# kosta777/parallel-genomeseq

Measured on AMD Instinct MI355X. Metric: GCUPS (cell updates/s), 150 bp reads vs 50 Mbp reference, whole job (score + argmax + traceback), higher is better.
Workload: dtype f16

## Files before the change

include/mi355_sw.h:

```cpp
#ifndef MI355_SW_H_
#define MI355_SW_H_

#include <stddef.h>
#include <stdint.h>

#ifdef __cplusplus
extern "C" {
#endif

enum { MI355_SW_F32 = 0, MI355_SW_U8SAT = 1 };

enum {
  MI355_SW_OK = 0,
  MI355_SW_EINVAL = -22,
  MI355_SW_ENOMEM = -12,
  MI355_SW_ENODEV = -19,
  MI355_SW_ENOTSUP = -95,
  MI355_SW_ERANGE = -34
};

enum {
  MI355_SW_SCORE_ONLY = 1
};

// ... 148 lines not shown
int mi355_sw_fill_matrix(mi355_sw_ctx *ctx, const char *x, size_t nx, const char *y, size_t ny,
                         const mi355_sw_params *params, float *H);

int mi355_sw_argmax(mi355_sw_ctx *ctx, const char *x, size_t nx, const char *y, size_t ny,
                    const mi355_sw_params *params, int64_t *index_x, int64_t *index_y, float *max);

int mi355_sw_last_timings(const mi355_sw_ctx *ctx, double out[6]);

int mi355_sw_last_counters(const mi355_sw_ctx *ctx, uint64_t out[4]);
int mi355_sw_last_counter(const mi355_sw_ctx *ctx, const char *name, uint64_t *out);

int mi355_sw_prefix_values(mi355_sw_ctx *ctx, float *values, size_t capacity, size_t *n_sub);

int mi355_sw_prefix_thin_items(mi355_sw_ctx *ctx, size_t n_items, const uint32_t *items, int P, int P2, int64_t sub_len, int64_t left, int64_t right,
                               const mi355_sw_params *params, float *values, size_t capacity, size_t *n_per_item);

int mi355_sw_seed_usable(const uint8_t *read, int32_t len, int k, const uint8_t *letters, size_t n_letters);
int mi355_sw_seed_certify_ok(int64_t d, int64_t smax, int64_t g, int64_t u);
int mi355_sw_seed_certify_window(int64_t start, int64_t m, int64_t d, int64_t smax, int64_t g, int64_t n, int64_t *lo, int64_t *hi);
int mi355_sw_seed_k(int letters, int min_len, int64_t n);
uint32_t mi355_sw_seed_hash(const uint8_t *codes, int k);
int mi355_sw_seed_cluster(size_t n_hits, const int64_t *starts, const int32_t *offsets, int64_t width, int64_t *lo, int64_t *hi, int *distinct);
int mi355_sw_seed_hits(mi355_sw_ctx *ctx, int64_t left, int64_t right, int k, uint32_t *counts, int64_t *starts, int32_t *offsets, int *k_used);

const char *mi355_sw_last_path(const mi355_sw_ctx *ctx);

enum {
  MI355_SW_CELL_I16 = 0,
  MI355_SW_CELL_U8 = 1,
  MI355_SW_CELL_F32 = 2,
  MI355_SW_CELL_F32U8 = 3,
  MI355_SW_CELL_F16 = 4,
  MI355_SW_CELL_U8H = 5
};
typedef struct {
  int cell;
  int lanes;
  int rows_per_lane;
  int strips;
  int twin;
  int64_t chunk_len;
  int64_t sub_len;
  int64_t warm;
  double cells;
  double valu_ops_per_cell;
  char name[160];
// ... 33 lines not shown
```

parallel-genomeseq_amd/capi.py:

```python
import ctypes as C
import os
import time

import numpy as np

_HERE = os.path.dirname(os.path.abspath(__file__))
LIB_PATH = os.path.join(_HERE, "libmi355_sw.so")

F32, U8SAT = 0, 1
SCORE_ONLY = 1

EXPORTS = [
    "mi355_sw_create", "mi355_sw_destroy", "mi355_sw_last_error", "mi355_sw_default_params",
    "mi355_sw_align", "mi355_sw_set_reference", "mi355_sw_align_batch", "mi355_sw_batch_upload",
    "mi355_sw_batch_run", "mi355_sw_score_ranges", "mi355_sw_align_scored_range", "mi355_sw_align_split", "mi355_sw_make_string_range", "mi355_sw_fill_matrix",
    "mi355_sw_argmax", "mi355_sw_true2raw", "mi355_sw_raw2true", "mi355_sw_last_timings", "mi355_sw_free_result", "mi355_sw_free_results",
    "mi355_sw_build_info", "mi355_sw_last_kernel", "mi355_sw_batch_run_view",
    "mi355_sw_multi_create", "mi355_sw_multi_destroy", "mi355_sw_multi_last_error", "mi355_sw_multi_device_count",
    "mi355_sw_multi_rccl_version", "mi355_sw_multi_align_split", "mi355_sw_multi_set_reference",
    "mi355_sw_multi_align_batch", "mi355_sw_multi_last_timings",
    "mi355_sw_set_option", "mi355_sw_option_names", "mi355_sw_multi_set_option", "mi355_sw_last_counters", "mi355_sw_last_counter", "mi355_sw_batch_upload_packed", "mi355_sw_best_range", "mi355_sw_last_path",
    "mi355_sw_default_affine_params", "mi355_sw_affine_align", "mi355_sw_affine_batch_run", "mi355_sw_affine_score_ranges",
    "mi355_sw_affine_align_trace", "mi355_sw_affine_batch_trace", "mi355_sw_affine_pairs_run", "mi355_sw_affine_pairs_trace",
    "mi355_sw_prefix_values", "mi355_sw_prefix_thin_items", "mi355_sw_affine_pairs_run_mode", "mi355_sw_affine_pairs_trace_mode",
    "mi355_sw_affine_pairs_run_band", "mi355_sw_affine_pairs_trace_band",
    "mi355_sw_affine_extend_run", "mi355_sw_affine_extend_trace",
    "mi355_sw_affine_extend_run_band", "mi355_sw_affine_extend_trace_band",
    "mi355_sw_affine_global_run", "mi355_sw_affine_global_trace",
    "mi355_sw_affine_extend_run_zdrop", "mi355_sw_affine_extend_trace_zdrop",
    "mi355_sw_seed_k", "mi355_sw_seed_hash", "mi355_sw_seed_cluster", "mi355_sw_seed_hits",
    "mi355_sw_seed_usable", "mi355_sw_seed_certify_ok", "mi355_sw_seed_certify_window",
]
SEED_HIT_CAP = 32
AFFINE_LOCAL, AFFINE_END_TO_END = 0, 1
AFFINE_MODES = {"local": AFFINE_LOCAL, "end_to_end": AFFINE_END_TO_END}
MULTI_RCCL = 1


class Params(C.Structure):
    _fields_ = [("lut", C.POINTER(C.c_float)), ("match", C.c_float), ("mismatch", C.c_float),
                ("gap", C.c_float), ("semantics", C.c_int)]


class AffineParams(C.Structure):
    _fields_ = [("lut", C.POINTER(C.c_float)), ("match", C.c_float), ("mismatch", C.c_float),
                ("gap_open", C.c_float), ("gap_extend", C.c_float)]


class ExtendList(C.Structure):
    _fields_ = [("npairs", C.c_size_t), ("query", C.POINTER(C.c_int32)), ("q_lo", C.POINTER(C.c_int32)), ("q_hi", C.POINTER(C.c_int32)),
                ("lefts", C.POINTER(C.c_int64)), ("rights", C.POINTER(C.c_int64)), ("backward", C.POINTER(C.c_uint8))]


class Result(C.Structure):
# ... 26 lines not shown

class MI355Error(RuntimeError):
    def __init__(self, code, msg):
        super().__init__("mi355_sw error %d: %s" % (code, msg))
        self.code = code


_LIB = None


def lib():
    global _LIB
    if _LIB is None:
        if not os.path.exists(LIB_PATH):
            raise ImportError("libmi355_sw.so not built: run `python -c 'import __graft_entry__ as g; g.build()'` "
                              "or `make -C parallel-genomeseq_amd/csrc`")
        L = C.CDLL(LIB_PATH)
        L.mi355_sw_last_error.restype = C.c_char_p
        L.mi355_sw_build_info.restype = C.c_char_p
        L.mi355_sw_multi_last_error.restype = C.c_char_p
        L.mi355_sw_option_names.restype = C.c_char_p
        L.mi355_sw_last_path.restype = C.c_char_p
        L.mi355_sw_seed_hash.restype = C.c_uint32
        for name in EXPORTS:
            getattr(L, name)
        _LIB = L
    return _LIB


def make_params(semantics=F32, match=3.0, mismatch=-3.0, gap=2.0, lut=None):
    p = Params()
    keep = None
    if lut is not None:
        keep = np.ascontiguousarray(lut, dtype=np.float32).reshape(65536)
        p.lut = keep.ctypes.data_as(C.POINTER(C.c_float))
    p.match, p.mismatch, p.gap, p.semantics = match, mismatch, gap, semantics
    return p, keep


def make_affine_params(match=3.0, mismatch=-3.0, gap_open=5.0, gap_extend=1.0, lut=None):
    p = AffineParams()
    keep = None
    if lut is not None:
        keep = np.ascontiguousarray(lut, dtype=np.float32).reshape(65536)
        p.lut = keep.ctypes.data_as(C.POINTER(C.c_float))
    p.match, p.mismatch, p.gap_open, p.gap_extend = match, mismatch, gap_open, gap_extend
# ... 477 lines not shown
            out[k] = np.array([r[k] for r in rows], dtype=np.int64)
        for k in ("cons_x", "cons_y", "cigar"):
            out[k] = [r[k] for r in rows]
        return out

    def align_batch(self, xs, y=None, **kw):
        if y is not None:
            self.set_reference(y)
        self.batch_upload(xs)
        return self.batch_run(**kw)

    def last_timings(self):
        t = (C.c_double * 6)()
        self._L.mi355_sw_last_timings(self._ctx, t)
        return dict(score_us=t[0], locate_us=t[1], trace_us=t[2], total_us=t[3], score_launches=int(t[4]), cells=t[5])


    def last_counters(self):
        c = (C.c_uint64 * 4)()
        self._L.mi355_sw_last_counters(self._ctx, c)
        out = dict(requeried=int(c[0]), whole_batch_again=int(c[1]), candidates=int(c[2]), left_window=int(c[3]))
        for name in ("first_settled", "saved_locates", "saved_traces", "saved_fallbacks", "walk_widened", "wait_retries", "early_settled", "beyond_f16", "prefix_certified",
                     "prefix_second_pass", "prefix_thinned", "prefix_thin_items", "pooled_loops", "prefix_seeded", "prefix_seed_hits", "prefix_calibrated", "seed_certified",
                     "zdrop_stopped", "zdrop_rows_run", "exact_launches", "trace_launches"):
            v = C.c_uint64(0)
            rc = self._L.mi355_sw_last_counter(self._ctx, name.encode(), C.byref(v))
            if rc:
                raise MI355Error(rc, "mi355_sw_last_counter(%s)" % name)
            out[name] = int(v.value)
        return out

    def prefix_values(self):
        nsub = C.c_size_t(0)
        self._chk(self._L.mi355_sw_prefix_values(self._ctx, None, C.c_size_t(0), C.byref(nsub)))
        if nsub.value == 0:
            return None
        out = np.zeros((self._nbatch, nsub.value), dtype=np.float32)
        self._chk(self._L.mi355_sw_prefix_values(self._ctx, out.ctypes.data_as(C.POINTER(C.c_float)), C.c_size_t(out.size), C.byref(nsub)))
        return out

    def prefix_thin_items(self, items, P, left, right, P2=38, sub_len=256, semantics=F32, match=3.0, mismatch=-3.0, gap=2.0, lut=None):
        p, keep = make_params(semantics, match, mismatch, gap, lut)
        flat = np.ascontiguousarray(np.asarray(items, dtype=np.uint32).reshape(-1, 2))
        per = C.c_size_t(0)
        args = (self._ctx, C.c_size_t(len(flat)), flat.ctypes.data_as(C.POINTER(C.c_uint32)), C.c_int(P), C.c_int(P2), C.c_int64(sub_len),
                C.c_int64(left), C.c_int64(right), C.byref(p))
        self._chk(self._L.mi355_sw_prefix_thin_items(*args, None, C.c_size_t(0), C.byref(per)))
# ... 141 lines not shown
def seed_usable(read, k, letters=b"ACGT"):
    x = np.ascontiguousarray(np.frombuffer(bytes(read), dtype=np.uint8))
    a = np.ascontiguousarray(np.frombuffer(bytes(letters), dtype=np.uint8))
    rc = lib().mi355_sw_seed_usable(x.ctypes.data_as(C.POINTER(C.c_uint8)), C.c_int32(len(x)), C.c_int(k),
                                    a.ctypes.data_as(C.POINTER(C.c_uint8)), C.c_size_t(len(a)))
    if rc < 0:
        raise MI355Error(rc, "mi355_sw_seed_usable")
    return int(rc)


def seed_certify_ok(d, smax, g, u):
    return bool(lib().mi355_sw_seed_certify_ok(C.c_int64(d), C.c_int64(smax), C.c_int64(g), C.c_int64(u)))


def seed_certify_window(start, m, d, smax, g, n):
    lo, hi = C.c_int64(0), C.c_int64(0)
    rc = lib().mi355_sw_seed_certify_window(C.c_int64(start), C.c_int64(m), C.c_int64(d), C.c_int64(smax), C.c_int64(g), C.c_int64(n),
                                            C.byref(lo), C.byref(hi))
    if rc < 0:
        raise MI355Error(rc, "mi355_sw_seed_certify_window")
    return (lo.value, hi.value) if rc == 1 else None


def seed_cluster(hits, width):
    starts = np.ascontiguousarray([h[0] for h in hits], dtype=np.int64)
    offs = np.ascontiguousarray([h[1] for h in hits], dtype=np.int32)
    lo, hi, d = C.c_int64(0), C.c_int64(0), C.c_int(0)
    rc = lib().mi355_sw_seed_cluster(C.c_size_t(len(starts)), starts.ctypes.data_as(C.POINTER(C.c_int64)), offs.ctypes.data_as(C.POINTER(C.c_int32)),
                                     C.c_int64(width), C.byref(lo), C.byref(hi), C.byref(d))
    if rc < 0:
        raise MI355Error(rc, "mi355_sw_seed_cluster")
    return (lo.value, hi.value, d.value) if rc == 1 else None
```

parallel-genomeseq_amd/csrc/host_common.h:

```cpp
namespace {

constexpr size_t kProfileLdsMax = 120 * 1024;
constexpr int kMaxRowsFast = 512;
constexpr size_t kDirsBudget = 16ull << 30;
constexpr size_t kExactLdsMax = 159 * 1024;

#define MI355_SW_BOOL_OPTIONS(X) \
  X(no_f16) X(no_unsat) X(no_sample) X(no_satflag) X(no_solo) X(no_wave) X(no_comb) X(no_twin) X(no_wide) X(no_strip) \
  X(no_quant) X(no_devlist) X(no_ref_cache) X(no_strip_groups) X(u8_long_twin) X(long_twin) X(no_long) \
  X(no_requery) X(force_f32) X(no_long_p32) X(no_opt_margin) X(no_wave_prof) X(no_wave_window) X(no_first) X(no_long_save) X(u8_sample_short) X(no_wave_pieces) X(no_u8_early) X(no_wave_f16) X(no_devlist_by_id) X(no_f16_mirror) X(no_f16m_int_diag) X(no_affine_sweep) X(no_affine_prof) X(no_affine_pairs) X(no_prefix) X(trace) \
  X(no_prefix_low) X(no_prefix_cascade) X(no_prefix_step) X(no_affine_band) X(no_prefix_thin) X(no_prefix_seed) X(no_seed_certify)
#define MI355_SW_INT_OPTIONS(X) X(strip_r) X(slot) X(few_r) X(chunk) X(long_pipes) X(long_wgs) X(long_sub) X(long_r) X(long_groups) X(assume_cus) X(long_save_what) X(prefix_min_cols) X(prefix_thin_min_cols) X(prefix_seed_min_cols) X(seed_certify_min_cols) X(seed_ride)
struct Options {
#define X(n) bool n = false;
  MI355_SW_BOOL_OPTIONS(X)
#undef X
#define X(n) long n = 0;
  MI355_SW_INT_OPTIONS(X)
#undef X
  bool prefix_tiles = false;
  long prefix_rowp = 0;
  long prefix_rowp_step = 0;
  bool prefix_thin_items = false;
  int fault_inject = 0;
};
inline std::string option_env_name(const char *n) {
  std::string e = "MI355_SW_";
  for (const char *c = n; *c; ++c) e += (char)std::toupper((unsigned char)*c);
  return e;
}
inline Options options_from_env() {
  Options o;
#define X(n) o.n = std::getenv(option_env_name(#n).c_str()) != nullptr;
  MI355_SW_BOOL_OPTIONS(X)
#undef X
// ... 292 lines not shown
  std::vector<uint16_t> h_atab;
  DevBuf aprof;
  std::vector<float> h_aprof;
  DevBuf rev_codes, rev_bytes, rev_q;
  bool rev_ref_valid = false, rev_q_valid = false;
  uint64_t rev_ref_version = 0, rev_q_version = 0;
  size_t rev_q_total = 0;
  std::vector<uint8_t> h_pieces;
  size_t saved_locates = 0, saved_traces = 0, saved_fallbacks = 0;
  size_t walk_widened = 0;
  size_t zdrop_stopped = 0;
  size_t zdrop_rows_run = 0;
  size_t exact_launches = 0;
  size_t trace_launches = 0;
  DevBuf thin_items, thin_out, thin_vals;
  DevBuf seed_tab, seed_hits;
  std::vector<uint8_t> h_qbytes;
  const void *h_qbytes_of = nullptr;
  uint64_t h_qbytes_version = 0;
  QueryBatch calib_q;
  PrefixBackground pbg;
  size_t prefix_seeded = 0;
  size_t seed_certified = 0;
  size_t prefix_seed_hits = 0;
  size_t prefix_calibrated = 0;
  DevBuf pkeys, pthr, psel, psel2, qcnt, sel2, gcnt, wlut, ckpt, first, keys, ranges, stab, ftab, ftab_s, htab, htab8, soloblk, flags, submax, lut, probs, dirs, outs_f, outs_i, cons, walkp, hmat, brow, wprobs, scan;
  std::vector<int64_t> h_ranges;
  std::vector<int16_t> h_stab;
  std::vector<float> h_ftab, h_ftab_s;
  int fshift = 0;
  std::vector<uint16_t> h_htab, h_htab8;
  std::vector<hipEvent_t> score_ev;
  size_t score_ev_used = 0;
  std::vector<std::vector<char>> arenas;
  PinBuf pin_probs, pin_walk, pin_out, pin_solo_up, pin_solo_down;
  std::vector<PinBuf> pin_cons;
  size_t cons_used = 0;
  double timings[6] = {0, 0, 0, 0, 0, 0};
  Options opts;
  ViewStore view;
  ScoredRanges scored;
  Helpers helpers;
  mi355_sw_kernel_info last_kernel = {};
};

namespace {

struct OptScope {
  const Options *prev;
  const DevInfo *prev_dev;
  explicit OptScope(const mi355_sw_ctx *c) : prev(tl_opt), prev_dev(tl_dev) {
    if (!prev) tl_pooled_loops = 0;
    if (c) { tl_opt = &c->opts; tl_dev = &c->dev; }
  }
  ~OptScope() { tl_opt = prev; tl_dev = prev_dev; if (!prev) tl_no_wait = false; }
};
// ... 430 lines not shown
```

parallel-genomeseq_amd/csrc/host_pipeline.h:

```cpp
namespace {

void set_result(mi355_sw_result &r, float score, int64_t ix, int64_t iy, const TraceOut *t) {
  r.score = score;
  r.end_x = score > 0 ? ix : 0;
  r.end_y = score > 0 ? iy : 0;
  r.pos = t ? t->pos : 0;
  const size_t len = t ? t->len : 0;
  r.cons_len = len;
  r.cons_x = (char *)malloc(2 * len + 2);
  r.cons_y = r.cons_x + len + 1;
  if (len) { memcpy(r.cons_x, t->cx, len); memcpy(r.cons_y, t->cy, len); }
  r.cons_x[len] = 0;
  r.cons_y[len] = 0;
}

int trace_located(mi355_sw_ctx *ctx, const RefData &ref, const QueryBatch &q, const Range &rg,
                  const mi355_sw_params &p, const std::vector<int64_t> &qwarm, const ScoreTable &table,
                  const std::vector<int> &qidx, const std::vector<Located> &loc, std::vector<TraceOut> &tout) {
  tout.assign(qidx.size(), TraceOut());
  const Margin mg = table.margin(q.maxlen);
  const float slope = (float)mg.slope();
  auto row_need = [&](int64_t i) { return mg.finite() ? clamp_cols((double)i + std::ceil((double)i * (double)slope) + 2.0) : kColsMax; };
  std::vector<size_t> todo;
  const bool wave_ok = wave_scoring_ok(p) && !opt().no_wave;
// ... 1879 lines not shown
  for (size_t k = 0; k < nq; ++k) if (!qfast[k]) slow.push_back((int)k);
  for (size_t r = 0; r < nr && !slow.empty(); ++r) {
    std::vector<Located> loc;
    std::vector<TraceOut> t;
    int rc = exact_full(ctx, ref, q, ranges[r], p, slow, false, loc, t);
    if (rc) return rc;
    for (size_t i = 0; i < slow.size(); ++i) maxima[r * nq + slow[i]] = loc[i].score;
  }
  sc.valid = keep;
  return 0;
}

int check_params(mi355_sw_ctx *ctx, const mi355_sw_params *p) {
  if (!ctx) return MI355_SW_EINVAL;
  if (!p) return fail(ctx, MI355_SW_EINVAL, "params is NULL");
  if (p->semantics != MI355_SW_F32 && p->semantics != MI355_SW_U8SAT) return fail(ctx, MI355_SW_EINVAL, "unknown semantics");
  return 0;
}

void reset_timings(mi355_sw_ctx *ctx) {
  for (double &t : ctx->timings) t = 0;
  ctx->score_ev_used = 0; ctx->arenas.clear(); ctx->cons_used = 0;
  ctx->last_kernel = mi355_sw_kernel_info{};
  ctx->requeried = 0; ctx->whole_again = 0; ctx->candidates = 0; ctx->prefix_certified = 0; ctx->prefix_second_pass = 0; ctx->prefix_thinned = 0; ctx->prefix_thin_items = 0; ctx->prefix_seeded = 0; ctx->prefix_seed_hits = 0; ctx->seed_certified = 0; ctx->prefix_calibrated = 0; ctx->prefix_named = false; ctx->left_window = 0; ctx->beyond_f16 = 0; ctx->first_settled = 0;
  ctx->hook_ids.clear(); ctx->hook_nsub = 0;
  ctx->saved_locates = 0; ctx->saved_traces = 0; ctx->saved_fallbacks = 0; ctx->walk_widened = 0; ctx->wait_retries = 0; ctx->early_settled = 0;
  ctx->zdrop_stopped = 0; ctx->zdrop_rows_run = 0;
  ctx->exact_launches = 0; ctx->trace_launches = 0;
  ctx->path.clear();
}

void reset_after_decline(mi355_sw_ctx *ctx) {
  const std::string ran = ctx->path;
  reset_timings(ctx);
  ctx->path = ran;
}

}
```

parallel-genomeseq_amd/csrc/host_score.h:

```cpp
namespace {

struct ScoreTable {
  bool ok = false;
  bool integral = false;
  std::string why;
  int gap = 0, smax = 0;
  float gapf = 0, smaxf = 0;
  std::vector<int16_t> stab;
  std::vector<uint16_t> htab;
  std::vector<uint16_t> htab8;
  std::vector<float> ftab;
  Margin margin(double rows) const { return make_margin(smaxf, gapf, integral, rows); }
};

struct Bucket {
  int first = 0, count = 0;
  int maxlen = 0;
  int R = 0;
  int SL = 16;
  int sem = kSemI16;
  bool strips = false;
  bool twin = false;
  bool comb = false;
  bool unsat = false;
// ... 348 lines not shown
  return true;
}

double valu_ops_per_cell(const Bucket &b) {
  const int R = b.R;
  const double over = b.SL == 8 ? 4.0 : 3.0;
  double per_step;
  int cells_per_row = 2;
  const int folded = b.sampled ? (R + sample_rows(b) - 1) / sample_rows(b) : R;
  double fold = (b.sampled ? 1.0 / kScoreMK : 1.0) * ((folded + 1) / 2);
  if (b.prefix && b.rowp && b.step) fold = 1.0;
  switch (b.sem) {
    case kSemF32:   per_step = 3.0 * R + (b.longp ? (b.sampled ? 1.0 / kLongMK : 1.0) * ((R + 1) / 2) : fold) + 1 + over; cells_per_row = 1; break;
    case kSemF32U8: per_step = 6.0 * R + (R + 1) / 2 + over; cells_per_row = 1; break;
    case kSemF16:   per_step = 3.0 * R + fold + 1 + over; break;
    case kSemU8H:   { const int odd = R / 2; per_step = 4.0 * R + odd / 2 + odd % 2 + R % 2 + over; break; }
    case kSemU8:    per_step = 5.0 * R + (R + 1) / 2 + R % 2 + over; break;
    default:        per_step = 4.0 * R + (R + 1) / 2 + R % 2 + over; break;
  }
  if (b.twin && !b.comb) per_step += R;
  return per_step / (double)(cells_per_row * R);
}

int launch_score(const ScoreInst &want, dim3 grid, size_t shmem, hipStream_t st, const ScoreArgs &a) {
  for (size_t k = 0; k < kScoreInsts.size(); ++k) {
    if (!(kScoreInsts[k] == want)) continue;
    if (shmem > 48 * 1024)
      (void)hipFuncSetAttribute(reinterpret_cast<const void *>(kScoreKernels[k]), hipFuncAttributeMaxDynamicSharedMemorySize, (int)shmem);
    hipLaunchKernelGGL(kScoreKernels[k], grid, dim3(256), shmem, st, a);
    return 0;
  }
  for (size_t k = 0; low_step_inst(want) && k < std::size(kR2Step); ++k) {
    if (kR2Step[k] != want.R) continue;
    if (shmem > 48 * 1024)
      (void)hipFuncSetAttribute(reinterpret_cast<const void *>(kLowStepKernels[k]), hipFuncAttributeMaxDynamicSharedMemorySize, (int)shmem);
    hipLaunchKernelGGL(kLowStepKernels[k], grid, dim3(256), shmem, st, a);
    return 0;
  }
  return -1;
}

int kernel_sem(const Bucket &b) {
  if (b.sem == kSemF16 && b.mirror) return opt().no_f16m_int_diag ? kSemF16MF : kSemF16M;
  return b.sem;
}

constexpr int64_t kPrefixMinCols = (int64_t)8 << 20;
constexpr int kPrefixProbe = 64;
inline int64_t prefix_cols_min() { const long v = opt().prefix_min_cols; return v > 0 ? (int64_t)v : kPrefixMinCols; }
float prefix_bound(const ScoreTable &t, int m, int P, float slack, bool rowp) {
  const float b = (float)t.smax * (float)(m - P) + slack;
  return rowp ? std::max(b, (float)t.smax * (float)P) : b;
}
bool prefix_height_ok(const ScoreTable &t, const Bucket &b, int minlen, int R, bool rowp, bool step = false) {
  const int P = kPrefixLanes * R;
  if (!(rowp && step ? prefix_step_listed(R) : listed(kR8M, R)) || minlen <= P) return false;
  return (float)t.smax * (float)minlen > prefix_bound(t, b.maxlen, P, rowp ? rowp_slack(t, rowp_mk(step)) : sample_slack(t, b), rowp);
}
bool prefix_ok(const ScoreTable &t, const Bucket &b, int minlen, int64_t n, const mi355_sw_params &p) {
  if (opt().no_prefix || p.semantics != MI355_SW_F32 || !t.integral || t.gap <= 0 || t.smax <= 0) return false;
  if (!(b.fast && b.sem == kSemF16 && b.mirror && b.sampled && !b.strips && !b.twin && !b.satflag && !b.unsat && b.SL == 8 && b.count >= 2)) return false;
  if (kernel_sem(b) != kSemF16M || !listed(kR8M, b.R)) return false;
// ... 91 lines not shown
    };
    auto cost = [&](int64_t c) { return rounds(c) * (double)(c + warm + SL); };
    const double r0 = rounds(cl);
    if (r0 <= 8.0) {
      const double need_rounds = std::min(2.0, r0);
      const double base = cost(cl);
      int64_t best = cl;
      double best_gain = 0.0;
      const int64_t lo = std::max<int64_t>({quant, floor_cl, (cl / 2 + quant - 1) / quant * quant});
      for (int64_t c = lo; c <= 2 * cl; c += quant) {
        const double rc = rounds(c);
        if (rc < need_rounds) continue;
        const double gain = 1.0 - cost(c) / base;
        if (gain < (rc < r0 ? 0.07 : 0.04)) continue;
        if (gain > best_gain) { best_gain = gain; best = c; }
      }
      cl = best;
    }
  }
  { const long v = opt().chunk; if (v >= 64) cl = v / 64 * 64; }
  return cl;
}

int score_tables(mi355_sw_ctx *ctx, int maxlen, int64_t maxrange, const ScoreTable &t) {
  const void *stab_was = ctx->stab.p, *ftab_was = ctx->ftab.p;
  if (ctx->stab.ensure(t.stab.size() * 2) || ctx->ftab.ensure(t.ftab.size() * 4 + 16))
    return fail(ctx, MI355_SW_ENOMEM, "hipMalloc(score scratch) failed");
  if (ctx->stab.p != stab_was || ctx->h_stab != t.stab) {
    ctx->h_stab = t.stab;
    HIPCHK(ctx, hipMemcpyAsync(ctx->stab.p, ctx->h_stab.data(), ctx->h_stab.size() * 2, hipMemcpyHostToDevice, ctx->stream));
  }
  if (!t.ftab.empty() && (ctx->ftab.p != ftab_was || ctx->h_ftab != t.ftab)) {
    ctx->h_ftab = t.ftab;
    HIPCHK(ctx, hipMemcpyAsync(ctx->ftab.p, ctx->h_ftab.data(), ctx->h_ftab.size() * 4, hipMemcpyHostToDevice, ctx->stream));
  }
  if (!t.ftab.empty()) {
    const double bound = (double)t.smaxf * (double)std::min<int64_t>(std::max(1, maxlen), std::max<int64_t>(1, maxrange)) + (double)t.smaxf + 1.0;
    ctx->fshift = std::max(1, std::min(100, std::ilogb(bound) + 2));
    std::vector<float> scaled(t.ftab.size());
    for (size_t k = 0; k < scaled.size(); ++k) scaled[k] = std::ldexp(t.ftab[k], -ctx->fshift);
    const void *was = ctx->ftab_s.p;
    if (ctx->ftab_s.ensure(scaled.size() * 4 + 16)) return fail(ctx, MI355_SW_ENOMEM, "hipMalloc(score scratch) failed");
    if (ctx->ftab_s.p != was || ctx->h_ftab_s != scaled) {
      ctx->h_ftab_s.swap(scaled);
      HIPCHK(ctx, hipMemcpyAsync(ctx->ftab_s.p, ctx->h_ftab_s.data(), ctx->h_ftab_s.size() * 4, hipMemcpyHostToDevice, ctx->stream));
    }
// ... 223 lines not shown
  }
  return 0;
}

int score_launch(mi355_sw_ctx *ctx, const RefData &ref, const QueryBatch &q, const std::vector<Range> &ranges,
                 const mi355_sw_params &p, const ScoreTable &t, Bucket &b, const ScoreIO *io = nullptr) {
  if (b.longp && io == nullptr) return long_score_launch(ctx, ref, q, ranges, p, t, b);
  HostTrace trace_("score_launch");
  const size_t nr = ranges.size();
  int64_t maxlen = 0;
  for (auto &r : ranges) maxlen = std::max(maxlen, r.hi - r.lo);
  const int sem = kernel_sem(b);
  const CellLaunch cl = cell_launch(ctx, t, sem);
  const int nqw = b.twin ? 1 : cl.queries;
  const size_t npairs = nqw == 1 ? (size_t)b.count : ((size_t)b.count + 1) / 2;
  b.sub_len = score_sub_len(p.semantics, b);
  const bool free_sub = p.semantics == MI355_SW_F32 && b.strips;
  if (b.strips && !free_sub) {
    const int64_t cl0 = pick_chunk_len(maxlen, npairs * nr, b.warm, b.SL, b.twin, b.maxlen, b.sub_len, 0);
    while (2 * cl0 / b.sub_len > 64) b.sub_len *= 2;
  }
  const bool chain_main = b.prefix && b.rowp && b.step && b.SL == kPrefixLanes && (b.bulk || (!b.second && b.count >= kPrefixChain - kPrefixProbe));
  b.chunk_len = pick_chunk_len(maxlen, npairs * nr, b.warm, b.SL, b.twin, b.maxlen, b.sub_len, free_sub ? 64 * kSeg : b.sub_len, chain_main);
  if (free_sub && b.chunk_len % (64 * kSeg) == 0) b.sub_len = b.chunk_len / 64;
  if (b.strips) while (b.chunk_len / b.sub_len > 64) b.sub_len *= 2;
  if (b.sub_len > b.chunk_len || b.chunk_len % b.sub_len != 0) b.sub_len = b.chunk_len;
  const int64_t cpr = (maxlen + b.chunk_len - 1) / b.chunk_len;
  const int nslot = 256 / b.SL;
  const int64_t cgroups = ((b.twin ? (cpr + 1) / 2 : cpr) + nslot - 1) / nslot;
  if ((double)npairs * (double)cgroups > 2.0e9) return fail(ctx, MI355_SW_ENOTSUP, "grid too large");

  ScoreArgs a;
  a.refcodes = ref.codes.as<uint8_t>();
  a.ref_len = (int64_t)ref.n;
  a.range_lo = io ? io->range_lo : ctx->ranges.as<int64_t>();
  a.range_hi = io ? io->range_hi : ctx->ranges.as<int64_t>() + nr;
  a.chunk_len = b.chunk_len;
  a.sub_len = b.sub_len;
  a.warm = (cpr == 1) ? 0 : b.warm;
  if (b.prefix && !b.strips && a.warm > 0) {
    const Margin pmg = t.margin(b.SL * b.R);
    if (pmg.finite()) a.warm = std::min(a.warm, (pmg.cols(b.SL * b.R) + 63) / 64 * 64);
  }
  a.chunks_per_range = (int)cpr;
  a.qbytes = q.bytes.as<uint8_t>();
  a.qoff = q.offs.as<int64_t>();
  a.qlen = q.lens.as<int32_t>();
  a.qsel = q.sel.as<int32_t>();
  a.qfirst = b.first;
  a.qcount = b.count;
  a.nq = (int)q.nq;
  a.stab = cl.tab;
  a.ncodes = ref.ncodes;
  a.gap2 = cl.gap2;
  a.clamp2 = 255u * 0x00010001u;
  a.pubmax = b.unsat ? cl.pubmax : 0u;
  a.keys = io ? io->keys : ctx->keys.as<unsigned long long>();
  a.flag_count = nullptr; a.flag_list = nullptr; a.flag_cap = 0; a.flag_value = 0;
  a.submax_out = nullptr; a.submax_stride = 0;
  if (b.sampled && nr != 1) b.sampled = false;
  if (b.satflag) {
    a.flag_count = ctx->flags.as<unsigned int>();
    a.flag_list = reinterpret_cast<uint2 *>(ctx->flags.as<unsigned int>() + 2);
    a.flag_cap = ctx->flag_cap;
    a.flag_value = (uint32_t)half_bits(1.0f);
  }
// ... 128 lines not shown
    case kKeyF32:       memcpy(&v, &hi, 4); return v;
    default:            return (float)hi;
  }
}

constexpr int kRetryNoWait = 1;

int score_fetch(mi355_sw_ctx *ctx, size_t count, std::vector<unsigned long long> &keys, const void *from = nullptr) {
  keys.resize(count);
  HIPCHK(ctx, hipMemcpyAsync(keys.data(), from ? from : ctx->keys.p, count * 8, hipMemcpyDeviceToHost, ctx->stream));
  int32_t long_status = 0;
  if (ctx->long_launched) HIPCHK(ctx, hipMemcpyAsync(&long_status, ctx->flags.as<unsigned int>() + 1, 4, hipMemcpyDeviceToHost, ctx->stream));
  HIPCHK(ctx, hipStreamSynchronize(ctx->stream));
  ctx->long_launched = false;
  if (long_status != 0) {
    ctx->score_ev_used = 0;
    if (!tl_no_wait) { tl_no_wait = true; ctx->wait_retries += 1; return kRetryNoWait; }
    return fail(ctx, MI355_SW_ENODEV, "sw_long_kernel: a pipeline wait expired (a wavefront of the workgroup made no progress)");
  }
  for (size_t e = 0; e + 1 < ctx->score_ev_used; e += 2) {
    float ms = 0;
    HIPCHK(ctx, hipEventElapsedTime(&ms, ctx->score_ev[e], ctx->score_ev[e + 1]));
    ctx->timings[0] += (double)ms * 1000.0;
  }
  ctx->score_ev_used = 0;
  return 0;
}

}
```

parallel-genomeseq_amd/csrc/mi355_sw.hip:

```cpp
#include "../../include/mi355_sw.h"

#include <hip/hip_runtime.h>

#include <algorithm>
#include <array>
#include <atomic>
#include <chrono>
#include <condition_variable>
#include <functional>
#include <iterator>
#include <map>
#include <future>
#include <mutex>
#include <thread>
#include <memory>
#include <cmath>
#include <cstdarg>
#include <cstdio>
#include <cstdlib>
#include <cstring>
#include <string>
#include <utility>
#include <vector>

// ... 723 lines not shown
  return 0;
}

int mi355_sw_last_counters(const mi355_sw_ctx *ctx, uint64_t out[4]) {
  if (!ctx || !out) return MI355_SW_EINVAL;
  out[0] = ctx->requeried; out[1] = ctx->whole_again; out[2] = ctx->candidates; out[3] = ctx->left_window;
  return 0;
}

int mi355_sw_last_counter(const mi355_sw_ctx *ctx, const char *name, uint64_t *out) {
  if (!ctx || !name || !out) return MI355_SW_EINVAL;
  const std::string k(name);
  if (k == "requeried") *out = ctx->requeried;
  else if (k == "whole_batch_again") *out = ctx->whole_again;
  else if (k == "candidates") *out = ctx->candidates;
  else if (k == "prefix_certified") *out = ctx->prefix_certified;
  else if (k == "prefix_second_pass") *out = ctx->prefix_second_pass;
  else if (k == "prefix_thinned") *out = ctx->prefix_thinned;
  else if (k == "prefix_thin_items") *out = ctx->prefix_thin_items;
  else if (k == "prefix_seeded") *out = ctx->prefix_seeded;
  else if (k == "prefix_seed_hits") *out = ctx->prefix_seed_hits;
  else if (k == "seed_certified") *out = ctx->seed_certified;
  else if (k == "prefix_calibrated") *out = ctx->prefix_calibrated;
  else if (k == "left_window") *out = ctx->left_window;
  else if (k == "beyond_f16") *out = ctx->beyond_f16;
  else if (k == "first_settled") *out = ctx->first_settled;
  else if (k == "wait_retries") *out = ctx->wait_retries;
  else if (k == "early_settled") *out = ctx->early_settled;
  else if (k == "saved_locates") *out = ctx->saved_locates;
  else if (k == "saved_traces") *out = ctx->saved_traces;
  else if (k == "saved_fallbacks") *out = ctx->saved_fallbacks;
  else if (k == "walk_widened") *out = ctx->walk_widened;
  else if (k == "zdrop_stopped") *out = ctx->zdrop_stopped;
  else if (k == "zdrop_rows_run") *out = ctx->zdrop_rows_run;
  else if (k == "exact_launches") *out = ctx->exact_launches;
  else if (k == "trace_launches") *out = ctx->trace_launches;
  else if (k == "pooled_loops") *out = tl_pooled_loops;
  else return MI355_SW_EINVAL;
  return 0;
}

int mi355_sw_prefix_values(mi355_sw_ctx *ctx, float *values, size_t capacity, size_t *n_sub) {
  if (!ctx || !n_sub) return MI355_SW_EINVAL;
  OptScope opt_scope_(ctx);
  const size_t nsub = (size_t)ctx->hook_nsub, nq = ctx->batch.nq;
  *n_sub = nsub;
// ... 55 lines not shown
  if ((n_hits && (!starts || !offsets)) || !lo || !hi || !distinct || width < 0) return MI355_SW_EINVAL;
  std::vector<SeedHit> hits(n_hits);
  for (size_t k = 0; k < n_hits; ++k) hits[k] = SeedHit{starts[k], offsets[k]};
  *lo = 0; *hi = 0; *distinct = 0;
  return seed_cluster(hits, width, *lo, *hi, *distinct) ? 1 : 0;
}

int mi355_sw_seed_usable(const uint8_t *read, int32_t len, int k, const uint8_t *letters, size_t n_letters) {
  if (!read || len < 0 || k < 1 || k > kSeedMaxK || (n_letters && !letters)) return MI355_SW_EINVAL;
  int code_of[256];
  for (int b = 0; b < 256; ++b) code_of[b] = -1;
  for (size_t i = 0; i < n_letters; ++i) code_of[letters[i]] = 0;
  const int64_t off = 0;
  const int32_t id = 0;
  SeedTable t;
  if (!seed_table_build(t, k, read, &off, &len, &id, 1, code_of)) return MI355_SW_ENOTSUP;
  std::vector<uint32_t> u;
  seed_usable(t, 1, u);
  return (int)u[0];
}

int mi355_sw_seed_certify_ok(int64_t d, int64_t smax, int64_t g, int64_t u) { return seed_certify_ok(d, smax, g, u) ? 1 : 0; }

int mi355_sw_seed_certify_window(int64_t start, int64_t m, int64_t d, int64_t smax, int64_t g, int64_t n, int64_t *lo, int64_t *hi) {
  if (!lo || !hi) return MI355_SW_EINVAL;
  *lo = 0; *hi = -1;
  int64_t a = 0, b = -1;
  if (!seed_certify_window(start, m, d, smax, g, n, a, b)) return 0;
  *lo = a; *hi = b;
  return 1;
}

int mi355_sw_seed_hits(mi355_sw_ctx *ctx, int64_t left, int64_t right, int k, uint32_t *counts, int64_t *starts, int32_t *offsets, int *k_used) {
  if (!ctx || !counts || !starts || !offsets) return MI355_SW_EINVAL;
  OptScope opt_scope_(ctx);
  const QueryBatch &q = ctx->batch;
  const RefData &ref = ctx->ref;
  if (left < 0 || right < left || right > (int64_t)ref.n) return fail(ctx, MI355_SW_EINVAL, "range outside the resident reference");
  if (q.nq == 0) return fail(ctx, MI355_SW_EINVAL, "mi355_sw_seed_hits: no resident batch");
  HIPCHK(ctx, hipSetDevice(ctx->device));
  if (k == 0) k = seed_k(ref.ncodes - 1, q.len[q.order[0]], right - left);
  if (k < 1 || k > kSeedMaxK) return fail(ctx, MI355_SW_ENOTSUP, "mi355_sw_seed_hits: no seed length for these reads and this range");
  if (k_used) *k_used = k;
  std::vector<int32_t> ids(q.nq);
  for (size_t i = 0; i < q.nq; ++i) ids[i] = (int32_t)i;
  std::vector<uint32_t> count;
// ... 32 lines not shown
```

Baseline: 886,500.

## Pick prefix-path tile length from occupancy-based wave-fill cost model

Adds a cost model that queries kernel occupancy (resident workgroups per CU) and chooses a smaller chunk length for the bulk prefix scoring path, so that workgroups fill the device's slots in fewer partial waves. Each candidate tile is costed as warm-up plus tile columns times rounds of workgroups, and the length only changes when the model predicts a sufficient saving. Smaller tiles raise the warm-up overhead per column, and the path only engages for references of at least 4M columns under particular bucket conditions. It also adds counters, trace output and C/Python exports for testing the model.

```diff
diff --git a/include/mi355_sw.h b/include/mi355_sw.h
--- a/include/mi355_sw.h
+++ b/include/mi355_sw.h
@@ -194,6 +194,10 @@
 uint32_t mi355_sw_seed_hash(const uint8_t *codes, int k);
 int mi355_sw_seed_cluster(size_t n_hits, const int64_t *starts, const int32_t *offsets, int64_t width, int64_t *lo, int64_t *hi, int *distinct);
 int mi355_sw_seed_hits(mi355_sw_ctx *ctx, int64_t left, int64_t right, int k, uint32_t *counts, int64_t *starts, int32_t *offsets, int *k_used);
+
+int64_t mi355_sw_prefix_group_tile_len(int64_t pairs, int64_t cols, int64_t sub_len, int64_t warm, int lanes, int cus, int resident,
+                                       int64_t old_len, double f0, double cap);
+void mi355_sw_prefix_fill_constants(double *f0, double *cap, double *gain);
 
 const char *mi355_sw_last_path(const mi355_sw_ctx *ctx);
 
diff --git a/parallel-genomeseq_amd/capi.py b/parallel-genomeseq_amd/capi.py
--- a/parallel-genomeseq_amd/capi.py
+++ b/parallel-genomeseq_amd/capi.py
@@ -30,6 +30,7 @@
     "mi355_sw_affine_extend_run_zdrop", "mi355_sw_affine_extend_trace_zdrop",
     "mi355_sw_seed_k", "mi355_sw_seed_hash", "mi355_sw_seed_cluster", "mi355_sw_seed_hits",
     "mi355_sw_seed_usable", "mi355_sw_seed_certify_ok", "mi355_sw_seed_certify_window",
+    "mi355_sw_prefix_group_tile_len", "mi355_sw_prefix_fill_constants",
 ]
 SEED_HIT_CAP = 32
 AFFINE_LOCAL, AFFINE_END_TO_END = 0, 1
@@ -102,6 +103,8 @@
         L.mi355_sw_option_names.restype = C.c_char_p
         L.mi355_sw_last_path.restype = C.c_char_p
         L.mi355_sw_seed_hash.restype = C.c_uint32
+        L.mi355_sw_prefix_group_tile_len.restype = C.c_int64
+        L.mi355_sw_prefix_fill_constants.restype = None
         for name in EXPORTS:
             getattr(L, name)
         _LIB = L
@@ -625,7 +628,7 @@
         out = dict(requeried=int(c[0]), whole_batch_again=int(c[1]), candidates=int(c[2]), left_window=int(c[3]))
         for name in ("first_settled", "saved_locates", "saved_traces", "saved_fallbacks", "walk_widened", "wait_retries", "early_settled", "beyond_f16", "prefix_certified",
                      "prefix_second_pass", "prefix_thinned", "prefix_thin_items", "pooled_loops", "prefix_seeded", "prefix_seed_hits", "prefix_calibrated", "seed_certified",
-                     "zdrop_stopped", "zdrop_rows_run", "exact_launches", "trace_launches"):
+                     "zdrop_stopped", "zdrop_rows_run", "exact_launches", "trace_launches", "prefix_fill_moved", "prefix_fill_resident"):
             v = C.c_uint64(0)
             rc = self._L.mi355_sw_last_counter(self._ctx, name.encode(), C.byref(v))
             if rc:
@@ -813,6 +816,17 @@
     return (lo.value, hi.value) if rc == 1 else None
 
 
+def prefix_group_tile_len(pairs, cols, sub_len, warm, lanes, cus, resident, old_len, f0=0.0, cap=0.0):
+    return int(lib().mi355_sw_prefix_group_tile_len(C.c_int64(pairs), C.c_int64(cols), C.c_int64(sub_len), C.c_int64(warm), C.c_int(lanes),
+                                                    C.c_int(cus), C.c_int(resident), C.c_int64(old_len), C.c_double(f0), C.c_double(cap)))
+
+
+def prefix_fill_constants():
+    f0, cap, gain = C.c_double(0), C.c_double(0), C.c_double(0)
+    lib().mi355_sw_prefix_fill_constants(C.byref(f0), C.byref(cap), C.byref(gain))
+    return f0.value, cap.value, gain.value
+
+
 def seed_cluster(hits, width):
     starts = np.ascontiguousarray([h[0] for h in hits], dtype=np.int64)
     offs = np.ascontiguousarray([h[1] for h in hits], dtype=np.int32)
diff --git a/parallel-genomeseq_amd/csrc/host_common.h b/parallel-genomeseq_amd/csrc/host_common.h
--- a/parallel-genomeseq_amd/csrc/host_common.h
+++ b/parallel-genomeseq_amd/csrc/host_common.h
@@ -9,8 +9,8 @@
   X(no_f16) X(no_unsat) X(no_sample) X(no_satflag) X(no_solo) X(no_wave) X(no_comb) X(no_twin) X(no_wide) X(no_strip) \
   X(no_quant) X(no_devlist) X(no_ref_cache) X(no_strip_groups) X(u8_long_twin) X(long_twin) X(no_long) \
   X(no_requery) X(force_f32) X(no_long_p32) X(no_opt_margin) X(no_wave_prof) X(no_wave_window) X(no_first) X(no_long_save) X(u8_sample_short) X(no_wave_pieces) X(no_u8_early) X(no_wave_f16) X(no_devlist_by_id) X(no_f16_mirror) X(no_f16m_int_diag) X(no_affine_sweep) X(no_affine_prof) X(no_affine_pairs) X(no_prefix) X(trace) \
-  X(no_prefix_low) X(no_prefix_cascade) X(no_prefix_step) X(no_affine_band) X(no_prefix_thin) X(no_prefix_seed) X(no_seed_certify)
-#define MI355_SW_INT_OPTIONS(X) X(strip_r) X(slot) X(few_r) X(chunk) X(long_pipes) X(long_wgs) X(long_sub) X(long_r) X(long_groups) X(assume_cus) X(long_save_what) X(prefix_min_cols) X(prefix_thin_min_cols) X(prefix_seed_min_cols) X(seed_certify_min_cols) X(seed_ride)
+  X(no_prefix_low) X(no_prefix_cascade) X(no_prefix_step) X(no_affine_band) X(no_prefix_thin) X(no_prefix_seed) X(no_seed_certify) X(no_prefix_fill)
+#define MI355_SW_INT_OPTIONS(X) X(strip_r) X(slot) X(few_r) X(chunk) X(long_pipes) X(long_wgs) X(long_sub) X(long_r) X(long_groups) X(assume_cus) X(long_save_what) X(prefix_min_cols) X(prefix_thin_min_cols) X(prefix_seed_min_cols) X(seed_certify_min_cols) X(seed_ride) X(prefix_fill_min_cols) X(prefix_group_chunk)
 struct Options {
 #define X(n) bool n = false;
   MI355_SW_BOOL_OPTIONS(X)
@@ -349,6 +349,8 @@
   PrefixBackground pbg;
   size_t prefix_seeded = 0;
   size_t seed_certified = 0;
+  size_t prefix_fill_moved = 0;
+  size_t prefix_fill_resident = 0;
   size_t prefix_seed_hits = 0;
   size_t prefix_calibrated = 0;
   DevBuf pkeys, pthr, psel, psel2, qcnt, sel2, gcnt, wlut, ckpt, first, keys, ranges, stab, ftab, ftab_s, htab, htab8, soloblk, flags, submax, lut, probs, dirs, outs_f, outs_i, cons, walkp, hmat, brow, wprobs, scan;
@@ -359,6 +361,7 @@
   std::vector<uint16_t> h_htab, h_htab8;
   std::vector<hipEvent_t> score_ev;
   size_t score_ev_used = 0;
+  std::map<std::pair<const void *, size_t>, int> score_resident;
   std::vector<std::vector<char>> arenas;
   PinBuf pin_probs, pin_walk, pin_out, pin_solo_up, pin_solo_down;
   std::vector<PinBuf> pin_cons;
diff --git a/parallel-genomeseq_amd/csrc/host_pipeline.h b/parallel-genomeseq_amd/csrc/host_pipeline.h
--- a/parallel-genomeseq_amd/csrc/host_pipeline.h
+++ b/parallel-genomeseq_amd/csrc/host_pipeline.h
@@ -1925,7 +1925,7 @@
   for (double &t : ctx->timings) t = 0;
   ctx->score_ev_used = 0; ctx->arenas.clear(); ctx->cons_used = 0;
   ctx->last_kernel = mi355_sw_kernel_info{};
-  ctx->requeried = 0; ctx->whole_again = 0; ctx->candidates = 0; ctx->prefix_certified = 0; ctx->prefix_second_pass = 0; ctx->prefix_thinned = 0; ctx->prefix_thin_items = 0; ctx->prefix_seeded = 0; ctx->prefix_seed_hits = 0; ctx->seed_certified = 0; ctx->prefix_calibrated = 0; ctx->prefix_named = false; ctx->left_window = 0; ctx->beyond_f16 = 0; ctx->first_settled = 0;
+  ctx->requeried = 0; ctx->whole_again = 0; ctx->candidates = 0; ctx->prefix_certified = 0; ctx->prefix_second_pass = 0; ctx->prefix_thinned = 0; ctx->prefix_thin_items = 0; ctx->prefix_seeded = 0; ctx->prefix_seed_hits = 0; ctx->seed_certified = 0; ctx->prefix_calibrated = 0; ctx->prefix_fill_moved = 0; ctx->prefix_fill_resident = 0; ctx->prefix_named = false; ctx->left_window = 0; ctx->beyond_f16 = 0; ctx->first_settled = 0;
   ctx->hook_ids.clear(); ctx->hook_nsub = 0;
   ctx->saved_locates = 0; ctx->saved_traces = 0; ctx->saved_fallbacks = 0; ctx->walk_widened = 0; ctx->wait_retries = 0; ctx->early_settled = 0;
   ctx->zdrop_stopped = 0; ctx->zdrop_rows_run = 0;
diff --git a/parallel-genomeseq_amd/csrc/host_score.h b/parallel-genomeseq_amd/csrc/host_score.h
--- a/parallel-genomeseq_amd/csrc/host_score.h
+++ b/parallel-genomeseq_amd/csrc/host_score.h
@@ -394,22 +394,36 @@
   return per_step / (double)(cells_per_row * R);
 }
 
+ScoreKernel score_kernel_of(const ScoreInst &want) {
+  for (size_t k = 0; k < kScoreInsts.size(); ++k)
+    if (kScoreInsts[k] == want) return kScoreKernels[k];
+  for (size_t k = 0; low_step_inst(want) && k < std::size(kR2Step); ++k)
+    if (kR2Step[k] == want.R) return kLowStepKernels[k];
+  return nullptr;
+}
+
 int launch_score(const ScoreInst &want, dim3 grid, size_t shmem, hipStream_t st, const ScoreArgs &a) {
-  for (size_t k = 0; k < kScoreInsts.size(); ++k) {
-    if (!(kScoreInsts[k] == want)) continue;
-    if (shmem > 48 * 1024)
-      (void)hipFuncSetAttribute(reinterpret_cast<const void *>(kScoreKernels[k]), hipFuncAttributeMaxDynamicSharedMemorySize, (int)shmem);
-    hipLaunchKernelGGL(kScoreKernels[k], grid, dim3(256), shmem, st, a);
-    return 0;
-  }
-  for (size_t k = 0; low_step_inst(want) && k < std::size(kR2Step); ++k) {
-    if (kR2Step[k] != want.R) continue;
-    if (shmem > 48 * 1024)
-      (void)hipFuncSetAttribute(reinterpret_cast<const void *>(kLowStepKernels[k]), hipFuncAttributeMaxDynamicSharedMemorySize, (int)shmem);
-    hipLaunchKernelGGL(kLowStepKernels[k], grid, dim3(256), shmem, st, a);
-    return 0;
-  }
-  return -1;
+  const ScoreKernel kernel = score_kernel_of(want);
+  if (!kernel) return -1;
+  if (shmem > 48 * 1024)
+    (void)hipFuncSetAttribute(reinterpret_cast<const void *>(kernel), hipFuncAttributeMaxDynamicSharedMemorySize, (int)shmem);
+  hipLaunchKernelGGL(kernel, grid, dim3(256), shmem, st, a);
+  return 0;
+}
+
+int score_resident(mi355_sw_ctx *ctx, const ScoreInst &want, size_t shmem) {
+  const ScoreKernel kernel = score_kernel_of(want);
+  if (!kernel) return 0;
+  const std::pair<const void *, size_t> key{reinterpret_cast<const void *>(kernel), shmem};
+  auto at = ctx->score_resident.find(key);
+  if (at != ctx->score_resident.end()) return at->second;
+  if (shmem > 48 * 1024)
+    (void)hipFuncSetAttribute(key.first, hipFuncAttributeMaxDynamicSharedMemorySize, (int)shmem);
+  int n = 0;
+  if (hipOccupancyMaxActiveBlocksPerMultiprocessor(&n, key.first, 256, shmem) != hipSuccess) { (void)hipGetLastError(); n = 0; }
+  n = std::max(0, n);
+  ctx->score_resident[key] = n;
+  return n;
 }
 
 int kernel_sem(const Bucket &b) {
@@ -547,6 +561,41 @@
   return cl;
 }
 
+constexpr double kPrefixFillF0 = 0.5;
+constexpr double kPrefixFillCap = 0.045;
+constexpr double kPrefixFillGain = 0.04;
+constexpr double kPrefixFillMaxRounds = 2.0;
+constexpr int64_t kPrefixFillMinCols = (int64_t)4 << 20;
+inline int64_t prefix_fill_cols_min() { const long v = opt().prefix_fill_min_cols; return v > 0 ? (int64_t)v : kPrefixFillMinCols; }
+struct PrefixFill { int64_t wgs = 0, slots = 0; double rounds = 0.0, cost = 0.0; };
+PrefixFill prefix_fill_cost(int64_t pairs, int64_t n, int64_t c, int64_t warm, int SL, int cus, int resident, double f0) {
+  PrefixFill f;
+  const int64_t tiles = (n + c - 1) / c, per_wg = 256 / SL;
+  f.wgs = pairs * ((tiles + per_wg - 1) / per_wg);
+  f.slots = (int64_t)cus * (int64_t)resident;
+  f.rounds = (double)f.wgs / (double)f.slots + f0;
+  f.cost = (double)((warm + c + SL + 63) / 64 * 64) * f.rounds;
+  return f;
+}
+int64_t prefix_group_tile_len(int64_t pairs, int64_t n, int64_t E, int64_t warm, int SL, int cus, int resident, int64_t old_len,
+                              double f0 = kPrefixFillF0, double cap = kPrefixFillCap) {
+  if (pairs < 1 || n < 1 || E < 1 || warm < 0 || SL < 1 || SL > 256 || cus < 1 || resident < 1 || old_len < E || !(f0 >= 0.0) || !(cap > 0.0))
+    return old_len;
+  int64_t lo = E;
+  while (lo <= old_len && (double)(warm + SL) >= cap * (double)lo) lo += E;
+  const PrefixFill before = prefix_fill_cost(pairs, n, old_len, warm, SL, cus, resident, f0);
+  if ((double)before.wgs > kPrefixFillMaxRounds * (double)before.slots) return old_len;
+  const double base = before.cost;
+  int64_t best = old_len;
+  double best_cost = base;
+  for (int64_t c = old_len / E * E; c >= lo; c -= E) {
+    if (c == old_len) continue;
+    const double cost = prefix_fill_cost(pairs, n, c, warm, SL, cus, resident, f0).cost;
+    if (cost < best_cost) { best_cost = cost; best = c; }
+  }
+  return best_cost <= (1.0 - kPrefixFillGain) * base ? best : old_len;
+}
+
 int score_tables(mi355_sw_ctx *ctx, int maxlen, int64_t maxrange, const ScoreTable &t) {
   const void *stab_was = ctx->stab.p, *ftab_was = ctx->ftab.p;
   if (ctx->stab.ensure(t.stab.size() * 2) || ctx->ftab.ensure(t.ftab.size() * 4 + 16))
@@ -816,6 +865,37 @@
   }
   const bool chain_main = b.prefix && b.rowp && b.step && b.SL == kPrefixLanes && (b.bulk || (!b.second && b.count >= kPrefixChain - kPrefixProbe));
   b.chunk_len = pick_chunk_len(maxlen, npairs * nr, b.warm, b.SL, b.twin, b.maxlen, b.sub_len, free_sub ? 64 * kSeg : b.sub_len, chain_main);
+  int64_t prefix_warm = b.warm;
+  if (b.prefix && !b.strips && prefix_warm > 0) {
+    const Margin pmg = t.margin(b.SL * b.R);
+    if (pmg.finite()) prefix_warm = std::min(prefix_warm, (pmg.cols(b.SL * b.R) + 63) / 64 * 64);
+  }
+  if (chain_main && b.bulk && nr == 1 && b.sub_len > 0 && b.chunk_len % b.sub_len == 0 && opt().chunk < 64) {
+    const int64_t old_len = b.chunk_len, E = b.sub_len;
+    const bool on = !opt().no_prefix_fill;
+    const int64_t forced = on && opt().prefix_group_chunk >= E
+                             ? std::min<int64_t>({(int64_t)opt().prefix_group_chunk / E * E, 64 * E, (maxlen + E - 1) / E * E}) : 0;
+    const bool fill = on && forced == 0 && maxlen >= prefix_fill_cols_min();
+    int resident = 0;
+    if (forced || fill) {
+      const ScoreInst inst{b.R, sem, false, b.SL, false, false, 1, true};
+      const size_t lds = profile_lds_bytes(ref.ncodes, b.R, b.SL, b.twin, b.comb) + (size_t)(256 / b.SL) * codebuf_bytes(b.SL);
+      resident = score_resident(ctx, inst, lds);
+    }
+    if (forced) b.chunk_len = forced;
+    else if (fill) {
+      b.chunk_len = prefix_group_tile_len((int64_t)npairs, maxlen, E, prefix_warm, b.SL, dev_cus(), resident, old_len);
+      if (b.chunk_len != old_len) ctx->prefix_fill_moved += 1;
+      if (!b.second) ctx->prefix_fill_resident = (size_t)resident;
+    }
+    if (opt().trace) {
+      PrefixFill f;
+      if (resident > 0) f = prefix_fill_cost((int64_t)npairs, maxlen, b.chunk_len, prefix_warm, b.SL, dev_cus(), resident, kPrefixFillF0);
+      else f.wgs = (int64_t)npairs * (((maxlen + b.chunk_len - 1) / b.chunk_len + 256 / b.SL - 1) / (256 / b.SL));
+      std::fprintf(stderr, "[mi355_sw] prefix fill: R=%d pairs=%zu tile=%lld workgroups=%lld slots=%lld rounds=%.2f old=%lld%s\n", b.R, npairs,
+                   (long long)b.chunk_len, (long long)f.wgs, (long long)f.slots, f.rounds, (long long)old_len, forced ? " (forced)" : "");
+    }
+  }
   if (free_sub && b.chunk_len % (64 * kSeg) == 0) b.sub_len = b.chunk_len / 64;
   if (b.strips) while (b.chunk_len / b.sub_len > 64) b.sub_len *= 2;
   if (b.sub_len > b.chunk_len || b.chunk_len % b.sub_len != 0) b.sub_len = b.chunk_len;
@@ -832,10 +912,7 @@
   a.chunk_len = b.chunk_len;
   a.sub_len = b.sub_len;
   a.warm = (cpr == 1) ? 0 : b.warm;
-  if (b.prefix && !b.strips && a.warm > 0) {
-    const Margin pmg = t.margin(b.SL * b.R);
-    if (pmg.finite()) a.warm = std::min(a.warm, (pmg.cols(b.SL * b.R) + 63) / 64 * 64);
-  }
+  if (a.warm > 0) a.warm = prefix_warm;
   a.chunks_per_range = (int)cpr;
   a.qbytes = q.bytes.as<uint8_t>();
   a.qoff = q.offs.as<int64_t>();
@@ -1010,6 +1087,7 @@
     float ms = 0;
     HIPCHK(ctx, hipEventElapsedTime(&ms, ctx->score_ev[e], ctx->score_ev[e + 1]));
     ctx->timings[0] += (double)ms * 1000.0;
+    if (opt().trace) std::fprintf(stderr, "[mi355_sw] score launch: %.3f ms on the device\n", ms);
   }
   ctx->score_ev_used = 0;
   return 0;
diff --git a/parallel-genomeseq_amd/csrc/mi355_sw.hip b/parallel-genomeseq_amd/csrc/mi355_sw.hip
--- a/parallel-genomeseq_amd/csrc/mi355_sw.hip
+++ b/parallel-genomeseq_amd/csrc/mi355_sw.hip
@@ -769,6 +769,8 @@
   else if (k == "prefix_seed_hits") *out = ctx->prefix_seed_hits;
   else if (k == "seed_certified") *out = ctx->seed_certified;
   else if (k == "prefix_calibrated") *out = ctx->prefix_calibrated;
+  else if (k == "prefix_fill_moved") *out = ctx->prefix_fill_moved;
+  else if (k == "prefix_fill_resident") *out = ctx->prefix_fill_resident;
   else if (k == "left_window") *out = ctx->left_window;
   else if (k == "beyond_f16") *out = ctx->beyond_f16;
   else if (k == "first_settled") *out = ctx->first_settled;
@@ -870,6 +872,17 @@
 
 int mi355_sw_seed_certify_ok(int64_t d, int64_t smax, int64_t g, int64_t u) { return seed_certify_ok(d, smax, g, u) ? 1 : 0; }
 
+int64_t mi355_sw_prefix_group_tile_len(int64_t pairs, int64_t cols, int64_t sub_len, int64_t warm, int lanes, int cus, int resident,
+                                       int64_t old_len, double f0, double cap) {
+  return prefix_group_tile_len(pairs, cols, sub_len, warm, lanes, cus, resident, old_len, f0 > 0.0 ? f0 : kPrefixFillF0, cap > 0.0 ? cap : kPrefixFillCap);
+}
+
+void mi355_sw_prefix_fill_constants(double *f0, double *cap, double *gain) {
+  if (f0) *f0 = kPrefixFillF0;
+  if (cap) *cap = kPrefixFillCap;
+  if (gain) *gain = kPrefixFillGain;
+}
+
 int mi355_sw_seed_certify_window(int64_t start, int64_t m, int64_t d, int64_t smax, int64_t g, int64_t n, int64_t *lo, int64_t *hi) {
   if (!lo || !hi) return MI355_SW_EINVAL;
   *lo = 0; *hi = -1;
```

New measurement: 932,800 (median of 6 runs). 1.05x the previous value.
